# heathsc/bs_call

Hardware: AMD Instinct MI355X
Metric: genome positions called/sec (higher is better)
Workload: dtype f64

## Files before the change

### bs_call_amd/csrc/prepdev.hip

```cpp
#include <hip/hip_runtime.h>
#include <stdint.h>

#include "../../include/bscall_amd.h"

#define FLT_QUAL 63u

struct bsc_prep_plan {
  uint64_t src;
  uint64_t ms;
  uint32_t rl0;
  uint32_t w0, wl;
  uint32_t nm;
  uint32_t mark_l, mark_r;
  uint32_t out_len;
  uint32_t present;
  uint32_t trim_l, trim_r;
};

struct bsc_prep_desc {
  uint64_t srcw;
  uint32_t pk;
  int32_t pc;
};
#define PD_PRESENT 1u
#define PD_EDITED 2u
#define PD_SLOW 8u

#define PREP_CNT_WORDS 8u
#define PREP_CNT_SLOTS 64u
#define PE_ORI 1u
#define PE_READ 2u
#define PE_LIST 4u
#define PE_SOFT_POS 6u
#define PE_SOFT_ILL 7u
#define PE_INDEL 8u
#define PE_CAP 9u
#define PE_PROF_CAP 10u
#define PE_PROF_RANGE 11u

struct prep_rd {
  uint32_t w0, wl;
};
__device__ static __forceinline__ void d_left_trim(prep_rd &r, uint32_t l) {
  if (l > 0) {
    if (l >= r.wl) r.wl = 0;
    else {
      r.w0 += l;
      r.wl -= l;
    }
  }
}
__device__ static __forceinline__ void d_right_trim(prep_rd &r, uint32_t l) {
  if (l > 0) {
    if (l >= r.wl) r.wl = 0;
    else r.wl -= l;
  }
}

__device__ static __forceinline__ uint32_t d_qual(const uint8_t *sp, uint32_t i, uint32_t rl0, uint32_t mark_l, uint32_t mark_r) {
  return (i < mark_l || i >= rl0 - mark_r) ? FLT_QUAL : (uint32_t)sp[i] >> 2;
}

__device__ static __forceinline__ uint32_t d_ld32(const uint8_t *p);
__device__ static uint32_t d_mean_qual(const uint8_t *sp, const prep_rd &r, uint32_t rl0, uint32_t mark_l, uint32_t mark_r) {
  const uint32_t lo = r.w0 > mark_l ? r.w0 : mark_l;
  const uint32_t e0 = r.w0 + r.wl, e1 = rl0 - mark_r;
  const uint32_t hi = e0 < e1 ? e0 : e1;
  uint32_t tot = 0, n = 0, i = lo;
#define MQ_DWORD(w_)                                                                                                                   \
  {                                                                                                                                    \
    const uint32_t q = ((w_) >> 2) & 0x3f3f3f3fu;                                                                                      \
    const uint32_t nz = ((q ^ 0x3f3f3f3fu) + 0x7f7f7f7fu) & 0x80808080u;  \
    n += (uint32_t)__popc(nz);                                                                                                         \
    tot = __builtin_amdgcn_sad_u8(q & ((nz >> 7) * 0xffu), 0u, tot);                                       \
  }
  for (; i + 16u <= hi; i += 16u) {
    uint4 v;
    __builtin_memcpy(&v, sp + i, 16);
    MQ_DWORD(v.x) MQ_DWORD(v.y) MQ_DWORD(v.z) MQ_DWORD(v.w)
  }
  for (; i + 4u <= hi; i += 4u) MQ_DWORD(d_ld32(sp + i))
#undef MQ_DWORD
  for (; i < hi; i++) {
    const uint32_t q = (uint32_t)sp[i] >> 2;
// ... 291 lines not shown
    if (n_overlap) atomicAdd(&slot[1], n_overlap);
  }
}

__device__ static __forceinline__ uint32_t d_marked(const uint8_t *sp, uint32_t i, uint32_t rl0, uint32_t mark_l, uint32_t mark_r) {
  const bool in_r = i >= rl0 - mark_r;
  const uint32_t b = sp[(in_r && 2u * i > rl0 - 1u) ? rl0 - 1u - i : i];
  return (i < mark_l || in_r) ? (b & 3u) | (FLT_QUAL << 2) : (uint32_t)sp[i];
}

struct bsc_prep_prof {
  const uint8_t *ref;
  uint32_t x, n_ref, cap, used0;
  const uint32_t *used_scan;
  unsigned long long *table;
};
__device__ static const uint8_t PROF_REF[64] = {
    0, 0, 0, 0, 0, 0, 0, 0, 0, 0, 0, 8, 0, 0, 0, 0, 0, 4, 4, 0, 4, 0, 0, 0, 0, 0, 0, 8, 0, 0, 0, 0,
    0, 0, 0, 8, 0, 0, 0, 0, 0, 0, 0, 0, 0, 0, 0, 0, 0, 0, 0, 0, 0, 0, 0, 0, 0, 0, 0, 0, 0, 0, 0, 0};
__device__ static __forceinline__ uint32_t d_profile_base(uint32_t bs_strand, uint32_t c) {
  const uint32_t q = c >> 2;
  if (q < 20u  || q >= FLT_QUAL || bs_strand > 2u) return 0u;
  return ((bs_strand == 0 ? 0x7A6Bu : (bs_strand == 1 ? 0x5A4Bu : 0x7869u)) >> (4u * (c & 3u))) & 15u;
}

#define PREP_WAVES 4
#define PREP_BATCH 4u
#define PROF_LDS 512u

__device__ static __forceinline__ void d_prof_base(const bsc_prep_prof &F, uint32_t *s_prof, uint32_t strand, uint32_t used_t, int64_t v,
                                                   int32_t orig, uint32_t byte) {
  const uint32_t xx = d_profile_base(strand, byte);
  if (xx && v + 1 < (int64_t)F.n_ref) {
    const uint32_t ra = v >= 1 ? F.ref[v - 1] : 0u, rb = v >= 0 ? F.ref[v] : 0u, rc = F.ref[v + 1];
    const uint32_t m_before = PROF_REF[((ra << 3) | rb) & 63u], m_after = PROF_REF[((rb << 3) | rc) & 63u];
    if ((((xx & m_after) | ((xx & m_before) >> 1)) >> 2) & 1u) {
      const uint32_t ix = (uint32_t)(orig + 1);
      if (ix < used_t && ix < F.cap) {
        if (ix < PROF_LDS) atomicAdd(&s_prof[(xx & 3u) * PROF_LDS + ix], 1u);
        else atomicAdd(&F.table[(uint64_t)ix * 4u + (xx & 3u)], 1ull);
      }
    }
  }
}

__device__ static __forceinline__ uint32_t d_bcast(uint32_t v, uint32_t l) { return (uint32_t)__builtin_amdgcn_readlane((int)v, (int)l); }
__device__ static __forceinline__ unsigned long long d_bcast64(unsigned long long v, uint32_t l) {
  return (unsigned long long)d_bcast((uint32_t)v, l) | ((unsigned long long)d_bcast((uint32_t)(v >> 32), l) << 32);
}
__device__ static __forceinline__ uint32_t d_ld32(const uint8_t *p) {
  uint32_t v;
  __builtin_memcpy(&v, p, 4);
  return v;
}
__device__ static __forceinline__ void d_st32(uint8_t *p, uint32_t v) { __builtin_memcpy(p, &v, 4); }

struct prep_slow_ret {
  uint32_t c63, cge;
  uint32_t walked;
};

__device__ static __forceinline__ uint32_t prep_slow_src(const bsc_prep_plan &P, const bsc_misms *__restrict__ ms, bool edited, uint32_t j, bool &pad) {
  uint32_t s = j;
  pad = false;
  if (edited) {
    for (uint32_t z = P.nm; z-- > 0;) {
      const bsc_misms m = ms[z];
      if (m.type == BSC_MISMS_INS) {
        if (s >= m.position) {
          if (s - m.position < m.size) {
            pad = true;
            break;
          }
          s -= m.size;
        }
      } else if (m.type == BSC_MISMS_DEL) {
        if (s >= m.position) s += m.size;
      }
    }
  }
  return s;
}

__device__ __noinline__ static prep_slow_ret prep_slow_read(const bsc_prep_plan *__restrict__ plan_r, uint32_t flags, uint8_t *__restrict__ dp,
                                                            const uint8_t *__restrict__ seq, const bsc_misms *__restrict__ ms_work, uint32_t mq) {
  const unsigned lane = threadIdx.x & 63u;
  prep_slow_ret r = {0u, 0u, 0u};
  const bsc_prep_plan P = *plan_r;
  const uint8_t *const sp = seq + P.src;
  const bool edited = (flags & PD_EDITED) != 0;
  if (edited) {
    for (uint32_t s0 = 0; s0 < P.wl; s0 += 64u) {
      const uint32_t s = s0 + lane;
      if (s < P.wl) {
        const uint32_t q = d_marked(sp, P.w0 + s, P.rl0, P.mark_l, P.mark_r) >> 2;
        r.c63 += q == FLT_QUAL;
        r.cge += q >= mq;
      }
    }
  }
  const bsc_misms *const ms = ms_work + P.ms;
  bool walked = false;
  for (uint32_t j0 = 0; j0 < P.out_len; j0 += 64u) {
    const uint32_t j = j0 + lane;
    if (j < P.out_len) {
      bool pad;
      const uint32_t s = prep_slow_src(P, ms, edited, j, pad);
      const uint32_t byte = pad ? 0u : d_marked(sp, P.w0 + s, P.rl0, P.mark_l, P.mark_r);
      const uint32_t q = byte >> 2;
      if (!edited) {
        r.c63 += q == FLT_QUAL;
        r.cge += q >= mq;
      }
      walked |= q != 0 && q != FLT_QUAL;
      dp[j] = (uint8_t)byte;
    }
  }
  r.walked = __any(walked) ? 1u : 0u;
  return r;
}

__global__ __launch_bounds__(64 * PREP_WAVES) void bsc_prep_copy_kernel(const bsc_prep_plan *__restrict__ plan,
                                                                        const bsc_prep_desc *__restrict__ desc, uint32_t nr,
                                                                        const uint8_t *__restrict__ seq, const bsc_misms *__restrict__ ms_work,
                                                                        const unsigned long long *__restrict__ out_off, int32_t min_qual,
                                                                        bsc_template *__restrict__ tpl_out, uint8_t *__restrict__ seq_out,
                                                                        uint64_t seq_out_cap, unsigned long long *__restrict__ cnt) {
  const unsigned lane = threadIdx.x & 63u, lane4 = lane * 4u;
  const uint32_t wave = (uint32_t)__builtin_amdgcn_readfirstlane((int)(blockIdx.x * PREP_WAVES + (threadIdx.x >> 6)));
  const uint32_t n_waves = gridDim.x * PREP_WAVES;
  const uint32_t mq = min_qual < 0 ? 0u : (min_qual > 64 ? 64u : (uint32_t)min_qual), mq4 = mq * 0x01010101u;
  unsigned long long l_total = 0, l_bases = 0;
  uint32_t c63 = 0, cge = 0, l_reads = 0;
  const uint32_t n_reads2 = 2u * nr, n_groups = (n_reads2 + 63u) / 64u;
  for (uint32_t g = wave; g < n_groups; g += n_waves) {
    const uint32_t g0 = g * 64u, n = n_reads2 - g0 < 64u ? n_reads2 - g0 : 64u;
    const uint32_t ri = g0 + (lane < n ? lane : 0u), my_ti = ri >> 1, my_k = ri & 1u;
    bsc_prep_desc L = desc[ri];
    const unsigned long long l_off = out_off[ri];
    if (lane >= n) L.pk = 0;
    if (lane < n) {
      const uint32_t fl = L.pk >> 28;
      uint32_t ol = L.pk & 0xfffffu, wl = ol;
      if (fl & PD_SLOW) {
        ol = plan[ri].out_len;
        wl = plan[ri].wl;
      }
      tpl_out[my_ti].off[my_k] = l_off;
      if (l_off > seq_out_cap || seq_out_cap - l_off < ol) {
        atomicMin(&cnt[0], ((unsigned long long)my_ti << 8) | PE_CAP);
        L.pk &= 0xf0000000u;
      }
      l_total += (fl & PD_EDITED) ? wl : ol;
      if (fl & PD_PRESENT) {
        l_reads++;
        l_bases += wl;
      }
    }
    enum : uint32_t { KIND_LEAN = 1u, KIND_FAST = 2u, KIND_SLOW = 3u };
    const uint32_t my_len = L.pk & 0xfffffu, my_ml = (L.pk >> 20) & 0xffu;
    const uint32_t my_kind = my_len == 0 ? 0u : ((L.pk >> 28) & PD_SLOW ? KIND_SLOW : ((my_len <= 256u && my_ml == 0) ? KIND_LEAN : KIND_FAST));
    const uint32_t l_ctl = (L.pk & 0x0fffffffu) | (my_kind << 28) | (((L.pk >> 28) & PD_EDITED) ? 1u << 30 : 0u);
    const bool my_fetch = my_kind == KIND_LEAN || my_kind == KIND_FAST;
    const unsigned long long l_src = my_fetch ? (unsigned long long)(seq + L.srcw) - (unsigned long long)desc : 0ull;
    unsigned long long walked_mask = 0;
    const unsigned long long obase = d_bcast64(l_off, 0);
    const unsigned long long m_w0 = __ballot(my_kind == KIND_LEAN && my_len >= 16u && my_len <= 128u);
    const unsigned long long sbase = m_w0 ? d_bcast64(L.srcw, (uint32_t)__builtin_ctzll(m_w0)) : 0ull;
    const unsigned long long orel = l_off - obase, srel = L.srcw - sbase;
    const bool my_wide = my_kind == KIND_LEAN && my_len >= 16u && my_len <= 128u && orel < (1ull << 24) && srel < (1ull << 31);
    const uint32_t w_a = my_wide ? my_len | ((uint32_t)orel << 8) : 0u, w_s = my_wide ? (uint32_t)srel : 0u;
    const uint32_t l16 = (lane & 7u) * 16u, sub = lane & 56u;
    const uint8_t *const sp_w = seq + sbase;
    uint8_t *const dp_w = seq_out + obase;
    uint32_t walk_bits = 0;
    constexpr uint32_t RW = 2u;
    auto fetch8 = [&](uint32_t i0, uint4(&vv)[RW]) {
#pragma unroll
      for (uint32_t i = 0; i < RW; i++) {
        const int src = (int)(sub | ((i0 + i) & 7u));
        const uint32_t len = (uint32_t)__shfl((int)w_a, src) & 0xffu, so = (uint32_t)__shfl((int)w_s, src);
        const uint32_t last = len ? len - 16u : 0u;
        __builtin_memcpy(&vv[i], sp_w + (so + (l16 < last ? l16 : last)), 16);
      }
    };
    auto process8 = [&](const uint32_t i0, const uint4(&v)[RW]) {
#pragma unroll
      for (uint32_t i = 0; i < RW; i++) {
        const uint32_t l = i0 + i;
        const int src = (int)(sub | l);
        const uint32_t a_ = (uint32_t)__shfl((int)w_a, src), len = a_ & 0xffu;
        const bool act = l16 < len;
        const uint32_t o = l16 < len - 16u ? l16 : len - 16u, dup = act ? l16 - o : 16u;
        const uint32_t w4[4] = {v[i].x, v[i].y, v[i].z, v[i].w};
        uint32_t any = 0;
#pragma unroll
        for (uint32_t d = 0; d < 4u; d++) {
          const uint32_t ge = (((0x83828180u + 0x04040404u * d) - dup * 0x01010101u) >> 7) & 0x01010101u;
          const uint32_t wc = w4[d] & (ge * 0xffu);
          const uint32_t qh = ((wc >> 2) & 0x3f3f3f3fu) | 0x80808080u;
          const uint32_t q1 = qh + 0x01010101u;
          c63 += (uint32_t)__popc(q1 & 0x40404040u);
          cge += (uint32_t)__popc((qh - mq4) & 0x80808080u);
          any |= q1 & 0x3e3e3e3eu;
        }
        if (any) walk_bits |= 1u << l;
        if (act) __builtin_memcpy(dp_w + ((a_ >> 8) + o), &v[i], 16);
      }
    };
    auto one = [&](const uint32_t l) {
      const uint32_t k = l & 1u;
      const uint32_t ctl = d_bcast(l_ctl, l), kind = (ctl >> 28) & 3u, len = ctl & 0xfffffu;
      uint8_t *const dp = seq_out + d_bcast64(l_off, l);
      if (kind == KIND_SLOW) {
        const prep_slow_ret r = prep_slow_read(plan + g0 + l, (ctl >> 30) & 1u ? PD_EDITED : 0u, dp, seq, ms_work, mq);
        c63 += r.c63;
        cge += r.cge;
        if (k == 0 && r.walked) walked_mask |= 1ull << l;
        return;
      }
      const uint32_t ml = (ctl >> 20) & 0xffu;
      bool walked = false;
      for (uint32_t base = 0; base < len; base += 256u) {
        const uint32_t nominal = base + lane4;
        const bool act = nominal < len;
        const uint32_t o = nominal < len - 4u ? nominal : len - 4u;
        uint32_t w = act ? d_ld32((const uint8_t *)desc + d_bcast64(l_src, l) + o) : 0u;
        if (ml + 3u > base) {
          const uint32_t nmk = act && ml > o ? (ml - o < 4u ? ml - o : 4u) : 0u;
          const uint32_t mm = nmk >= 4u ? 0xffffffffu : (1u << (8u * nmk)) - 1u;
          w = (w & ~mm) | (((w & 0x03030303u) | 0xfcfcfcfcu) & mm);
        }
        const uint32_t wc = act ? w >> (8u * (nominal - o)) : 0u;
        const uint32_t qh = ((wc >> 2) & 0x3f3f3f3fu) | 0x80808080u;
        const uint32_t q1 = qh + 0x01010101u;
        c63 += (uint32_t)__popc(q1 & 0x40404040u);
        cge += (uint32_t)__popc((qh - mq4) & 0x80808080u);
        if (k == 0) walked |= __any((q1 & 0x3e3e3e3eu) != 0u) != 0;
        if (act) d_st32(dp + o, w);
      }
      if (k == 0 && walked) walked_mask |= 1ull << l;
    };
    if (__ballot(my_wide)) {
      uint4 va[RW], vb[RW];
      fetch8(0, va);
#pragma unroll
      for (uint32_t i0 = 0; i0 < 8u; i0 += 2u * RW) {
        fetch8(i0 + RW, vb);
        process8(i0, va);
        fetch8(i0 + 2u * RW, va);
        process8(i0 + RW, vb);
      }
      walk_bits |= (uint32_t)__shfl_xor((int)walk_bits, 1);
      walk_bits |= (uint32_t)__shfl_xor((int)walk_bits, 2);
      walk_bits |= (uint32_t)__shfl_xor((int)walk_bits, 4);
      walked_mask |= __ballot((walk_bits >> (lane & 7u)) & 1u);
    }
    for (unsigned long long rest = __ballot(my_kind != 0u && !my_wide); rest; rest &= rest - 1ull) one((uint32_t)__builtin_ctzll(rest));
    if (lane < n && my_k == 0) tpl_out[my_ti].flags = BSC_TPL_WALK_KNOWN | (((walked_mask >> lane) & 1ull) ? BSC_TPL_WALKED0 : 0u);
  }
  unsigned long long w[5] = {l_total, c63, cge, l_reads, l_bases};
  for (int i = 0; i < 5; i++)
    for (int o = 32; o > 0; o >>= 1) w[i] += __shfl_xor(w[i], o);
  if (mq == 0) w[2] = w[0];
  if (lane == 0) {
    const unsigned long long low = w[0] - w[2] - (mq > FLT_QUAL ? w[1] : 0ull), none = w[0] - w[1] - low;
    if (none) atomicAdd(&cnt[3], none);
    if (w[1]) atomicAdd(&cnt[4], w[1]);
    if (low) atomicAdd(&cnt[5], low);
    if (w[3]) atomicAdd(&cnt[6], w[3]);
    if (w[4]) atomicAdd(&cnt[7], w[4]);
  }
}

__global__ __launch_bounds__(256) void bsc_prep_refmask_kernel(const uint8_t *__restrict__ ref, uint32_t n_ref, uint8_t *__restrict__ mask) {
  const uint64_t i = ((uint64_t)blockIdx.x * 256u + threadIdx.x) * 4u;
  if (i >= (uint64_t)n_ref + 24u) return;
  uint32_t m = 0;
  if (i >= 12u && i - 8u + 7u <= n_ref) {
    const uint64_t v = i - 8u;
    const uint32_t lo = d_ld32(ref + v - 1u) & 0x07070707u, hi = d_ld32(ref + v + 3u) & 0x07070707u;
    const uint32_t r_at = __builtin_amdgcn_alignbyte(hi, lo, 1u), r_next = __builtin_amdgcn_alignbyte(hi, lo, 2u);
#define PROF_NE(x, c) ((((x) ^ ((c) * 0x01010101u)) + 0x7f7f7f7fu) & 0x80808080u)
    const uint32_t over_c = ~PROF_NE(r_at, 2u) & PROF_NE(r_next, 0u) & PROF_NE(r_next, 3u) & 0x80808080u;
    const uint32_t over_g = ~PROF_NE(r_at, 3u) & PROF_NE(lo, 0u) & PROF_NE(lo, 2u) & 0x80808080u;
#undef PROF_NE
    m = (over_c >> 5) | (over_g >> 4);
  } else {
    for (uint32_t t = 0; t < 4u; t++) {
      const uint64_t it = i + t;
      if (it >= 8u && it - 8u + 1u < n_ref) {
        const uint64_t v = it - 8u;
        const uint32_t ra = v >= 1 ? ref[v - 1] : 0u, rb = ref[v], rc = ref[v + 1];
        m |= ((PROF_REF[((rb << 3) | rc) & 63u] & 4u) | (PROF_REF[((ra << 3) | rb) & 63u] & 8u)) << (8u * t);
      }
    }
  }
  __builtin_memcpy(mask + i, &m, 4);
}

__global__ __launch_bounds__(64 * PREP_WAVES) void bsc_prep_profile_kernel(const bsc_prep_plan *__restrict__ plan, const bsc_prep_desc *__restrict__ desc,
                                                                           uint32_t nr, const bsc_misms *__restrict__ ms_work,
                                                                           const unsigned long long *__restrict__ out_off,
                                                                           const bsc_template *__restrict__ tpl_out, const uint8_t *__restrict__ seq_out,
                                                                           uint64_t seq_out_cap, unsigned long long *__restrict__ cnt,
                                                                           const uint8_t *__restrict__ mask, const bsc_prep_prof F) {
  __shared__ uint32_t s_prof[PROF_LDS * 4u];
  for (unsigned i = threadIdx.x; i < PROF_LDS * 4u; i += 64 * PREP_WAVES) s_prof[i] = 0;
  __syncthreads();
  const unsigned lane = threadIdx.x & 63u;
  const uint32_t wave = (uint32_t)__builtin_amdgcn_readfirstlane((int)(blockIdx.x * PREP_WAVES + (threadIdx.x >> 6)));
  const uint32_t n_waves = gridDim.x * PREP_WAVES;
  const uint32_t n_reads2 = 2u * nr, n_groups = (n_reads2 + 63u) / 64u;
  uint32_t acc[4][2] = {{0u, 0u}, {0u, 0u}, {0u, 0u}, {0u, 0u}};
  uint32_t acc_n = 0;
  bool acc_quarter = true;
  auto flush = [&]() {
    const uint32_t p0 = 8u * (acc_quarter ? (lane & 15u) : (lane & 31u));
#pragma unroll
    for (uint32_t b = 0; b < 4u; b++) {
      const uint32_t col = (0x63u >> (2u * b)) & 3u;
#pragma unroll
      for (uint32_t t = 0; t < 8u; t++) {
        const uint32_t c = (acc[b][t >> 2] >> (8u * (t & 3u))) & 0xffu;
        if (c) atomicAdd(&s_prof[col * PROF_LDS + p0 + t + 1u], c);
      }
      acc[b][0] = acc[b][1] = 0u;
    }
    acc_n = 0;
  };
  for (uint32_t g = wave; g < n_groups; g += n_waves) {
    const uint32_t g0 = g * 64u, n = n_reads2 - g0 < 64u ? n_reads2 - g0 : 64u;
    const uint32_t ri = g0 + (lane < n ? lane : 0u), my_ti = ri >> 1, my_k = ri & 1u;
    const bsc_prep_desc L = desc[ri];
    const unsigned long long l_off = out_off[ri];
    const uint32_t us_prev = my_ti ? F.used_scan[my_ti - 1u] : 0u, us_mine = F.used_scan[my_ti];
    const uint32_t t_strand = tpl_out[my_ti].bs_strand, t_pos = tpl_out[my_ti].pos[my_k];
    uint32_t c1 = 0, kind = 0, l_used = 0, l_strand = 0, l_ol = 0, top = 0;
    if (lane < n) {
      const uint32_t fl = L.pk >> 28;
      uint32_t ol = L.pk & 0xfffffu;
// ... 81 lines not shown
      };
      rnd ra[B], rb[B];
#pragma unroll
      for (uint32_t u = 0; u < B; u++) ask(u, ra[u]);
      for (uint32_t i0 = 0; i0 < rounds; i0 += 2u * B) {
        if (acc_n + 2u * B > 255u) flush();
#pragma unroll
        for (uint32_t u = 0; u < B; u++) ask(i0 + B + u, rb[u]);
#pragma unroll
        for (uint32_t u = 0; u < B; u++) count(u, ra[u]);
#pragma unroll
        for (uint32_t u = 0; u < B; u++) ask(i0 + 2u * B + u, ra[u]);
#pragma unroll
        for (uint32_t u = 0; u < B; u++) count(B + u, rb[u]);
        acc_n += 2u * B;
      }
    }
    unsigned long long m_long = __ballot(kind == 2u);
    while (m_long) {
      const uint32_t l = (uint32_t)__builtin_ctzll(m_long);
      m_long &= m_long - 1ull;
      const uint32_t ol = d_bcast(l_ol, l), k = l & 1u, strand = d_bcast(l_strand, l), used_t = d_bcast(l_used, l);
      const int32_t pc = (int32_t)d_bcast((uint32_t)L.pc, l);
      const int64_t v0 = (int64_t)d_bcast(c1, l) - 1;
      const uint8_t *const dp = seq_out + d_bcast64(l_off, l);
      const bool slow = (d_bcast(L.pk, l) >> 28) & PD_SLOW;
      bsc_prep_plan P;
      bool edited = false;
      if (slow) {
        P = plan[g0 + l];
        edited = (d_bcast(L.pk, l) >> 28) & PD_EDITED;
      }
      for (uint32_t jb = 0; jb < ol; jb += 64u) {
        const uint32_t j = jb + lane;
        if (j < ol) {
          bool pad = false;
          const uint32_t s = slow ? prep_slow_src(P, ms_work + P.ms, edited, j, pad) : j;
          if (!pad) d_prof_base(F, s_prof, strand, used_t, v0 + j, k ? pc - (int32_t)s : pc + (int32_t)s, dp[j]);
        }
      }
    }
  }
  flush();
  __syncthreads();
  for (unsigned i = threadIdx.x; i < PROF_LDS * 4u; i += 64 * PREP_WAVES)
    if (s_prof[i] && i % PROF_LDS < F.cap) atomicAdd(&F.table[(uint64_t)(i % PROF_LDS) * 4u + i / PROF_LDS], (unsigned long long)s_prof[i]);
}

extern "C" int bsc_dev_scan_u64(const void *in, void *out, uint32_t n, void *tmp, size_t tmp_bytes, void *stream);

extern "C" size_t bsc_dev_prep_plan_bytes(void) { return sizeof(bsc_prep_plan) + sizeof(bsc_prep_desc); }

extern "C" int bsc_dev_scan_max_u32(const void *in, void *out, uint32_t n, void *tmp, size_t tmp_bytes, void *stream);

extern "C" int bsc_dev_launch_prep(const void *raw, uint32_t nr, const void *seq, uint64_t seq_bytes, const void *misms, uint64_t n_misms,
                                   const bsc_prep_params *par, void *ms_work, void *plan, void *out_len, void *out_off, void *scan_tmp,
                                   size_t scan_tmp_bytes, void *tpl_out, void *seq_out, uint64_t seq_out_cap, void *cnt, int num_cus,
                                   void *stream, const void *prof_ref, uint32_t prof_x, uint32_t prof_n_ref, uint32_t prof_cap,
                                   uint32_t prof_used0, void *prof_table, void *max_pos1, void *used_scan, void *prof_mask) {
  hipStream_t s = (hipStream_t)stream;
  bsc_prep_desc *const desc = (bsc_prep_desc *)((bsc_prep_plan *)plan + 2ull * nr);
  if (!nr) return (int)hipMemsetAsync(out_off, 0, sizeof(unsigned long long), s);
  hipError_t e = hipMemsetAsync((unsigned long long *)out_len + 2ull * nr, 0, sizeof(unsigned long long), s);
  if (e != hipSuccess) return (int)e;
  hipLaunchKernelGGL(bsc_prep_plan_kernel, dim3((nr + 255u) / 256u), dim3(256), 0, s, (const bsc_raw_template *)raw, nr, (const uint8_t *)seq,
                     seq_bytes, (const bsc_misms *)misms, n_misms, *par, (bsc_misms *)ms_work, (bsc_prep_plan *)plan, desc,
                     (unsigned long long *)out_len, (bsc_template *)tpl_out, (unsigned long long *)cnt, prof_ref ? (uint32_t *)max_pos1 : nullptr);
  if ((e = hipGetLastError()) != hipSuccess) return (int)e;
  int rc = bsc_dev_scan_u64(out_len, out_off, 2u * nr + 1u, scan_tmp, scan_tmp_bytes, stream);
  if (rc) return rc;
  bsc_prep_prof F = {nullptr, 0u, 0u, 0u, 0u, nullptr, nullptr};
  if (prof_ref) {
    if ((rc = bsc_dev_scan_max_u32(max_pos1, used_scan, nr, scan_tmp, scan_tmp_bytes, stream))) return rc;
    F.ref = (const uint8_t *)prof_ref;
    F.x = prof_x;
    F.n_ref = prof_n_ref;
    F.cap = prof_cap;
    F.used0 = prof_used0;
    F.used_scan = (const uint32_t *)used_scan;
    F.table = (unsigned long long *)prof_table;
  }
  unsigned g = ((nr + 31u) / 32u + PREP_WAVES - 1u) / PREP_WAVES;
  static int per_cu[2] = {0, 0};
  for (int pv = 0; pv < (prof_ref ? 2 : 1); pv++)
    if (!per_cu[pv]) {
      int nb = 0;
      const hipError_t eo = pv ? hipOccupancyMaxActiveBlocksPerMultiprocessor(&nb, bsc_prep_profile_kernel, 64 * PREP_WAVES, 0)
                               : hipOccupancyMaxActiveBlocksPerMultiprocessor(&nb, bsc_prep_copy_kernel, 64 * PREP_WAVES, 0);
      per_cu[pv] = (eo == hipSuccess && nb > 0) ? nb : 4;
      (void)hipGetLastError();
    }
  unsigned gc = g, gp = g;
  if (gc > (unsigned)num_cus * (unsigned)per_cu[0]) gc = (unsigned)num_cus * (unsigned)per_cu[0];
  hipLaunchKernelGGL(bsc_prep_copy_kernel, dim3(gc), dim3(64 * PREP_WAVES), 0, s, (const bsc_prep_plan *)plan, (const bsc_prep_desc *)desc, nr,
                     (const uint8_t *)seq, (const bsc_misms *)ms_work, (const unsigned long long *)out_off, par->min_qual, (bsc_template *)tpl_out,
                     (uint8_t *)seq_out, seq_out_cap, (unsigned long long *)cnt);
  if ((e = hipGetLastError()) != hipSuccess) return (int)e;
  if (prof_ref) {
    hipLaunchKernelGGL(bsc_prep_refmask_kernel, dim3((unsigned)(((uint64_t)prof_n_ref + 24u + 1023u) / 1024u)), dim3(256), 0, s, (const uint8_t *)prof_ref,
                       prof_n_ref, (uint8_t *)prof_mask);
    if ((e = hipGetLastError()) != hipSuccess) return (int)e;
    if (gp > (unsigned)num_cus * (unsigned)per_cu[1]) gp = (unsigned)num_cus * (unsigned)per_cu[1];
    hipLaunchKernelGGL(bsc_prep_profile_kernel, dim3(gp), dim3(64 * PREP_WAVES), 0, s, (const bsc_prep_plan *)plan, (const bsc_prep_desc *)desc, nr,
                       (const bsc_misms *)ms_work, (const unsigned long long *)out_off, (const bsc_template *)tpl_out, (const uint8_t *)seq_out,
                       seq_out_cap, (unsigned long long *)cnt, (const uint8_t *)prof_mask, F);
  }
  return (int)hipGetLastError();
}
```

### bs_call_amd/csrc/kernels.hip

```cpp
#include <hip/hip_runtime.h>
#include <stdint.h>

#include "bsmath.h"
#include "callmath.h"
#include "devtables.h"
#include "synth.h"

#ifndef TILE
#define TILE 256
#endif
#ifndef BSC_TILES_PER_WAVE
#define BSC_TILES_PER_WAVE 16
#endif
#ifndef BSC_WAVES_PER_SIMD
#define BSC_WAVES_PER_SIMD 4
#endif

template <bool FULL>
__global__ __launch_bounds__(TILE, BSC_WAVES_PER_SIMD) void bsc_call_kernel_t(const uint32_t *__restrict__ cts,
                                                                      const uint8_t *__restrict__ ref,
                                                                      uint64_t n_sites, uint64_t wt_begin,
                                                                      uint64_t wt_end, uint32_t *__restrict__ out,
                                                                      uint32_t out_dw, uint8_t *__restrict__ skip,
                                                                      const bsc_dev_tables *__restrict__ tb,
                                                                      uint32_t *__restrict__ het_list,
                                                                      unsigned long long *__restrict__ counters) {
  __shared__ __attribute__((aligned(16))) uint32_t lds_slot[TILE / 64][SLOT_DW];
  __shared__ double s_k[44], s_lnk[44], s_half[44], s_one[44];
#ifdef BSC_TABLES_GLOBAL
  const double *const s_logtab = tb->log_tab;
  const unsigned long long *const s_exptab = tb->exp_tab;
#else
  __shared__ double s_logtab[256];
  __shared__ unsigned long long s_exptab[256];
#endif
  __shared__ unsigned int s_cnt[12];
  __shared__ double s_ptab[PT_WORDS];
  __shared__ uint8_t s_pairs[TILE / 64][256];

  const unsigned tid = threadIdx.x;
  const unsigned lane = tid & 63u;
  const unsigned wid = __builtin_amdgcn_readfirstlane(tid >> 6);
  if (tid < 44) {
    s_k[tid] = tb->k[tid];
    s_lnk[tid] = tb->ln_k[tid];
    s_half[tid] = tb->ln_k_half[tid];
    s_one[tid] = tb->ln_k_one[tid];
  }
#ifndef BSC_TABLES_GLOBAL
  for (unsigned i = tid; i < 256; i += TILE) {
    s_logtab[i] = tb->log_tab[i];
    s_exptab[i] = tb->exp_tab[i];
  }
#endif
  if (tid < 12) s_cnt[tid] = 0;
  const double l = 1.0 - tb->under_conv;
  const double t = tb->over_conv;
  const double lrb = tb->lrb, lrb1 = tb->lrb1;
  __syncthreads();
  for (unsigned i = tid; i < PT_WORDS; i += TILE) s_ptab[i] = pure_log_entry(i, l, t, s_k, s_logtab);
  __syncthreads();

  uint32_t *slot = lds_slot[wid];
  const uint32_t wave_stride = gridDim.x * (TILE / 64);
  const uint32_t wt_last = (uint32_t)wt_end;
  for (uint32_t wt = (uint32_t)wt_begin + blockIdx.x * (TILE / 64) + wid; wt < wt_last; wt += wave_stride) {
    const uint64_t site0 = (uint64_t)wt * 64;
    const unsigned nvalid = FULL ? 64u : (unsigned)((n_sites - site0) < 64 ? (n_sites - site0) : 64);
    const bool full = FULL;
    const uint64_t site = site0 + lane;
    const bool valid = FULL || lane < nvalid;
    const unsigned rf = valid ? ref[site] : 0u;

    uint32_t w[IN_DW];
    if (full) {
      const char *src = reinterpret_cast<const char *>(cts + site0 * IN_DW) + lane * 16;
#pragma unroll
      for (int j = 0; j < 6; j++) dma16(src + j * 1024, slot + j * 256);
      if (lane < 32) dma16(src + 6 * 1024, slot + 6 * 256);
      asm volatile("s_waitcnt vmcnt(0)" ::: "memory");
      const uint2 *rec = reinterpret_cast<const uint2 *>(slot + lane * IN_DW);
#pragma unroll
      for (int i = 0; i < IN_DW / 2; i++) {
        const uint2 v = rec[i];
        w[2 * i] = v.x;
        w[2 * i + 1] = v.y;
      }
    } else {
#pragma unroll
      for (int i = 0; i < IN_DW; i++) w[i] = valid ? cts[site * IN_DW + i] : 0u;
    }
#include "call_body.inc"
    const bool het = covered && ((0x16Eu >> mxi) & 1u);
    if (covered) {
      atomicAdd(&s_cnt[0], 1u);
      atomicAdd(&s_cnt[1 + mxi], 1u);
    }
    {
      const unsigned long long m = __ballot(het);
      if (lane == 0) {
        reinterpret_cast<unsigned long long *>(het_list)[wt] = m;
        if (m) atomicAdd(&s_cnt[11], (unsigned)__popcll(m));
      }
    }
    if (valid) skip[site] = covered ? 0 : 1;

#pragma unroll 1
    for (unsigned half = 0; half < 2; half++) {
      __builtin_amdgcn_wave_barrier();
      const bool mine = valid && (lane >> 5) == half;
      auto write_record = [&](auto *rec) {
        if (covered) {
#pragma unroll
          for (int j = 0; j < 8; j++) rec[j] = make_uint2(cnt[j], 0u);
          rec[8] = make_uint2(qpack0 & 0xffu, (qpack0 >> 8) & 0xffu);
          rec[9] = make_uint2((qpack0 >> 16) & 0xffu, qpack0 >> 24);
          rec[10] = make_uint2(qpack1 & 0xffu, (qpack1 >> 8) & 0xffu);
          rec[11] = make_uint2((qpack1 >> 16) & 0xffu, qpack1 >> 24);
#pragma unroll
          for (int g = 0; g < 10; g++) {
            const uint64_t b = bsm_bits(gp[g]);
            rec[12 + g] = make_uint2((uint32_t)b, (uint32_t)(b >> 32));
          }
          rec[22] = make_uint2(0u, 0u);
          rec[23] = make_uint2((uint32_t)mq, (uint32_t)aq);
          rec[24] = make_uint2((uint32_t)mxi, 0u);
        } else {
#pragma unroll
          for (int j = 0; j < 25; j++) rec[j] = make_uint2(0u, 0u);
        }
        if (out_dw > OUT_DW) rec[25] = make_uint2(covered ? 0u : 0x100u, 0u);
      };
      if (mine) {
        if (full) write_record(reinterpret_cast<uint2 *>(slot + (lane & 31u) * out_dw));
        else write_record(reinterpret_cast<uint2 *>(out + site * out_dw));
      }
      if (full) {
        __builtin_amdgcn_wave_barrier();
        const unsigned nvec = 32u * out_dw / 4u;
        uint4 *dst = reinterpret_cast<uint4 *>(out + (site0 + half * 32u) * out_dw);
        const uint4 *srcv = reinterpret_cast<const uint4 *>(slot);
#pragma unroll
        for (unsigned v = 0; v < 7; v++) {
          const unsigned idx = v * 64u + lane;
          if (idx < nvec) {
            typedef unsigned int u32x4 __attribute__((ext_vector_type(4)));
            __builtin_nontemporal_store(reinterpret_cast<const u32x4 *>(srcv)[idx], reinterpret_cast<u32x4 *>(dst) + idx);
          }
        }
      }
    }
  }

  __syncthreads();
  if (tid < 12 && s_cnt[tid]) atomicAdd(&counters[BSC_CNT_COVERED + tid], (unsigned long long)s_cnt[tid]);
}

#define FI_THREADS 256
#define FI_LIST 2048
extern "C" __global__ __launch_bounds__(FI_THREADS) void bsc_fisher_kernel(const uint32_t *__restrict__ cts,
                                                                           uint32_t *__restrict__ out, uint32_t out_dw,
                                                                           const bsc_dev_tables *__restrict__ tb,
                                                                           const unsigned long long *__restrict__ masks,
                                                                           uint32_t n_tiles, uint32_t chunk_tiles) {
  __shared__ double s_lf[256];
  __shared__ double s_logtab[256];
  __shared__ unsigned long long s_exptab[256];
  __shared__ uint32_t s_scan[FI_THREADS + 1];
  __shared__ uint32_t s_list[FI_LIST];
  const unsigned tid = threadIdx.x;
  s_lf[tid] = tb->lfact[tid];
  s_logtab[tid] = tb->log_tab[tid];
  s_exptab[tid] = tb->exp_tab[tid];
  const uint32_t per = (chunk_tiles + FI_THREADS - 1) / FI_THREADS;
  for (uint32_t c0 = blockIdx.x * chunk_tiles; c0 < n_tiles; c0 += gridDim.x * chunk_tiles) {
    const uint32_t c1 = min(c0 + chunk_tiles, n_tiles);
    const uint32_t t0 = min(c0 + tid * per, c1), t1 = min(t0 + per, c1);
    uint32_t mine = 0;
    for (uint32_t t = t0; t < t1; t++) mine += (uint32_t)__popcll(masks[t]);
    __syncthreads();
    s_scan[tid + 1] = mine;
    if (tid == 0) s_scan[0] = 0;
    __syncthreads();
    if (tid < 64) {
      uint32_t a = s_scan[4 * tid + 1], b = a + s_scan[4 * tid + 2], c = b + s_scan[4 * tid + 3], d = c + s_scan[4 * tid + 4];
      uint32_t run = d;
#pragma unroll
      for (int off = 1; off < 64; off <<= 1) {
        const uint32_t v = __shfl_up(run, off);
        if ((int)tid >= off) run += v;
      }
      const uint32_t base = run - d;
      s_scan[4 * tid + 1] = base + a;
      s_scan[4 * tid + 2] = base + b;
      s_scan[4 * tid + 3] = base + c;
      s_scan[4 * tid + 4] = base + d;
    }
    __syncthreads();
    const uint32_t total = s_scan[FI_THREADS], first = s_scan[tid];
    for (uint32_t w0 = 0; w0 < total; w0 += FI_LIST) {
      if (w0) __syncthreads();
      if (first < w0 + FI_LIST && first + mine > w0) {
        uint32_t k = first;
        for (uint32_t t = t0; t < t1; t++) {
          unsigned long long m = masks[t];
          while (m) {
            const unsigned bit = (unsigned)__builtin_ctzll(m);
            m &= m - 1ull;
            if (k >= w0 && k < w0 + FI_LIST) s_list[k - w0] = t * 64u + bit;
            k++;
          }
        }
      }
      __syncthreads();
      const uint32_t cnt = min((uint32_t)FI_LIST, total - w0);
      for (uint32_t i = tid; i < cnt; i += FI_THREADS) {
        const uint64_t site = s_list[i];
        const uint32_t *p = cts + site * IN_DW;
        uint32_t f[8], r[8];
#pragma unroll
        for (int j = 0; j < 8; j++) {
          f[j] = p[j];
          r[j] = p[8 + j];
        }
        uint32_t *rec = out + site * out_dw;
        const unsigned mxi = rec[48] & 0xffu;
        int t0_, t1_, t2_, t3_;
        strand_table(mxi, f, r, t0_, t1_, t2_, t3_);
        double z = fisher_dev(t0_, t1_, t2_, t3_, s_lf, s_logtab, (const uint64_t *)s_exptab);
        if (z < 1.0e-20) z = 1.0e-20;
        const double fs = bsm_log_t(z, s_logtab) / BSM_LN10;
        const uint64_t b = bsm_bits(fs);
        reinterpret_cast<uint2 *>(rec)[22] = make_uint2((uint32_t)b, (uint32_t)(b >> 32));
      }
    }
  }
}

extern "C" __global__ __launch_bounds__(256) void bsc_synth_kernel(uint64_t seed, uint64_t first_site, uint64_t n,
                                                                   uint32_t coverage, uint32_t flags,
                                                                   uint32_t *__restrict__ cts,
                                                                   uint8_t *__restrict__ ref) {
  for (uint64_t i = (uint64_t)blockIdx.x * blockDim.x + threadIdx.x; i < n; i += (uint64_t)gridDim.x * blockDim.x) {
    uint32_t counts[16], nr, rf;
    float q[8], m2;
    syn_site(seed, first_site + i, coverage, flags, counts, &nr, q, &m2, &rf);
    uint32_t *p = cts + i * IN_DW;
#pragma unroll
    for (int j = 0; j < 16; j++) p[j] = counts[j];
    p[16] = nr;
#pragma unroll
    for (int j = 0; j < 8; j++) p[17 + j] = __float_as_uint(q[j]);
    p[25] = __float_as_uint(m2);
    ref[i] = (uint8_t)rf;
  }
}


extern "C" int bsc_dev_launch_call(const void *cts, const void *ref, uint64_t n, void *out, uint32_t out_dw, void *skip,
                                   const void *tb, void *het_list, void *counters, int num_cus, void *stream,
                                   void *ev_start, void *ev_mid, void *ev_stop) {
  if (n == 0) return 0;
  hipStream_t s = (hipStream_t)stream;
  if (ev_start) (void)hipEventRecord((hipEvent_t)ev_start, s);
  uint64_t resident = (uint64_t)num_cus * (BSC_WAVES_PER_SIMD * 4) / (TILE / 64);
  if (resident < 1) resident = 1;
  const uint64_t n_full = n / 64;
  hipError_t e = hipSuccess;
  if (n_full) {
    const uint64_t n_tiles = (n_full + (TILE / 64) - 1) / (TILE / 64);
    uint64_t rounds = n_full / (resident * (TILE / 64) * BSC_TILES_PER_WAVE);
    rounds = rounds < 1 ? 1 : (rounds > 16 ? 16 : rounds);
    uint64_t grid = resident * rounds;
    if (grid > n_tiles) grid = n_tiles;
    hipLaunchKernelGGL(bsc_call_kernel_t<true>, dim3((unsigned)grid), dim3(TILE), 0, s, (const uint32_t *)cts,
                       (const uint8_t *)ref, n, (uint64_t)0, n_full, (uint32_t *)out, out_dw, (uint8_t *)skip,
                       (const bsc_dev_tables *)tb, (uint32_t *)het_list, (unsigned long long *)counters);
    e = hipGetLastError();
    if (e != hipSuccess) return (int)e;
  }
  if (n & 63u) {
    hipLaunchKernelGGL(bsc_call_kernel_t<false>, dim3(1), dim3(TILE), 0, s, (const uint32_t *)cts, (const uint8_t *)ref, n,
                       n_full, n_full + 1, (uint32_t *)out, out_dw, (uint8_t *)skip, (const bsc_dev_tables *)tb,
                       (uint32_t *)het_list, (unsigned long long *)counters);
    e = hipGetLastError();
    if (e != hipSuccess) return (int)e;
  }
  if (ev_mid) (void)hipEventRecord((hipEvent_t)ev_mid, s);
  {
    const uint32_t n_tiles = (uint32_t)((n + 63) / 64);
    const uint32_t grid = (uint32_t)num_cus * 2u;
    uint32_t chunk = (n_tiles + grid - 1) / grid;
    chunk = chunk < 64u ? 64u : (chunk > 4096u ? 4096u : chunk);
    const uint32_t n_chunks = (n_tiles + chunk - 1) / chunk;
    hipLaunchKernelGGL(bsc_fisher_kernel, dim3(n_chunks < grid ? n_chunks : grid), dim3(FI_THREADS), 0, s, (const uint32_t *)cts,
                       (uint32_t *)out, out_dw, (const bsc_dev_tables *)tb, (const unsigned long long *)het_list, n_tiles, chunk);
  }
  e = hipGetLastError();
  if (ev_stop) (void)hipEventRecord((hipEvent_t)ev_stop, s);
  return (int)e;
}

extern "C" int bsc_dev_launch_synth(uint64_t seed, uint64_t first_site, uint64_t n, uint32_t coverage, uint32_t flags,
                                    void *cts, void *ref, int num_cus, void *stream) {
  if (n == 0) return 0;
  uint64_t grid = (n + 255) / 256;
  const uint64_t cap = (uint64_t)num_cus * 32u;
  if (grid > cap) grid = cap;
  hipLaunchKernelGGL(bsc_synth_kernel, dim3((unsigned)grid), dim3(256), 0, (hipStream_t)stream, seed, first_site, n,
                     coverage, flags, (uint32_t *)cts, (uint8_t *)ref);
  return (int)hipGetLastError();
}
```

Baseline: 16.75 billion.

## Stage per-wave output bytes in LDS and flush with aligned nontemporal stores

Each wave now assembles its group's output sequence bytes in a per-wave LDS image instead of scattering unaligned 4- and 16-byte global stores. After the group is built, the image is written to global memory in aligned 16-byte nontemporal chunks, with byte-wise handling at the edges. The host sizes the stage buffer from the mean read length and available LDS, and recomputes occupancy for the grid. The kernel also gains a waves-per-EU attribute and sched barriers. This costs LDS, may reduce occupancy, and adds a wave-level flush pass.

```diff
diff --git a/bs_call_amd/csrc/prepdev.hip b/bs_call_amd/csrc/prepdev.hip
--- a/bs_call_amd/csrc/prepdev.hip
+++ b/bs_call_amd/csrc/prepdev.hip
@@ -1,5 +1,7 @@
 #include <hip/hip_runtime.h>
 #include <stdint.h>
+
+#include <type_traits>
 
 #include "../../include/bscall_amd.h"
 
@@ -457,7 +459,15 @@
   return s;
 }
 
-__device__ __noinline__ static prep_slow_ret prep_slow_read(const bsc_prep_plan *__restrict__ plan_r, uint32_t flags, uint8_t *__restrict__ dp,
+extern __shared__ uint4 s_prep_stage[];
+#define PREP_NO_IMG 0xffffffffu
+#define PREP_LDS __attribute__((address_space(3)))
+typedef PREP_LDS uint8_t prep_lds_u8;
+typedef uint32_t __attribute__((aligned(1))) prep_u32_any;
+typedef unsigned int prep_u32x4 __attribute__((ext_vector_type(4)));
+typedef prep_u32x4 __attribute__((aligned(1))) prep_u32x4_any;
+
+__device__ __noinline__ static prep_slow_ret prep_slow_read(const bsc_prep_plan *__restrict__ plan_r, uint32_t flags, uint8_t *__restrict__ dp, uint32_t img,
                                                             const uint8_t *__restrict__ seq, const bsc_misms *__restrict__ ms_work, uint32_t mq) {
   const unsigned lane = threadIdx.x & 63u;
   prep_slow_ret r = {0u, 0u, 0u};
@@ -488,20 +498,24 @@
         r.cge += q >= mq;
       }
       walked |= q != 0 && q != FLT_QUAL;
-      dp[j] = (uint8_t)byte;
+      if (img != PREP_NO_IMG) ((prep_lds_u8 *)s_prep_stage)[img + j] = (uint8_t)byte;
+      else dp[j] = (uint8_t)byte;
     }
   }
   r.walked = __any(walked) ? 1u : 0u;
   return r;
 }
 
-__global__ __launch_bounds__(64 * PREP_WAVES) void bsc_prep_copy_kernel(const bsc_prep_plan *__restrict__ plan,
+__global__ __launch_bounds__(64 * PREP_WAVES) __attribute__((amdgpu_waves_per_eu(6))) void bsc_prep_copy_kernel(const bsc_prep_plan *__restrict__ plan,
                                                                         const bsc_prep_desc *__restrict__ desc, uint32_t nr,
                                                                         const uint8_t *__restrict__ seq, const bsc_misms *__restrict__ ms_work,
                                                                         const unsigned long long *__restrict__ out_off, int32_t min_qual,
                                                                         bsc_template *__restrict__ tpl_out, uint8_t *__restrict__ seq_out,
-                                                                        uint64_t seq_out_cap, unsigned long long *__restrict__ cnt) {
+                                                                        uint64_t seq_out_cap, unsigned long long *__restrict__ cnt,
+                                                                        uint32_t stage_bytes) {
   const unsigned lane = threadIdx.x & 63u, lane4 = lane * 4u;
+  const uint32_t img0 = (threadIdx.x >> 6) * stage_bytes;
+  prep_lds_u8 *const img = (prep_lds_u8 *)s_prep_stage + img0;
   const uint32_t wave = (uint32_t)__builtin_amdgcn_readfirstlane((int)(blockIdx.x * PREP_WAVES + (threadIdx.x >> 6)));
   const uint32_t n_waves = gridDim.x * PREP_WAVES;
   const uint32_t mq = min_qual < 0 ? 0u : (min_qual > 64 ? 64u : (uint32_t)min_qual), mq4 = mq * 0x01010101u;
@@ -540,6 +554,10 @@
     const unsigned long long l_src = my_fetch ? (unsigned long long)(seq + L.srcw) - (unsigned long long)desc : 0ull;
     unsigned long long walked_mask = 0;
     const unsigned long long obase = d_bcast64(l_off, 0);
+    const unsigned long long gend = out_off[g0 + n];
+    const uint32_t ia = (uint32_t)((unsigned long long)(seq_out + obase) & 15ull);
+    const bool staged = __builtin_amdgcn_readfirstlane((int)(gend <= seq_out_cap && gend >= obase && gend - obase + ia <= stage_bytes)) != 0;
+    const uint32_t span = staged ? (uint32_t)(gend - obase) : 0u;
     const unsigned long long m_w0 = __ballot(my_kind == KIND_LEAN && my_len >= 16u && my_len <= 128u);
     const unsigned long long sbase = m_w0 ? d_bcast64(L.srcw, (uint32_t)__builtin_ctzll(m_w0)) : 0ull;
     const unsigned long long orel = l_off - obase, srel = L.srcw - sbase;
@@ -559,7 +577,8 @@
         __builtin_memcpy(&vv[i], sp_w + (so + (l16 < last ? l16 : last)), 16);
       }
     };
-    auto process8 = [&](const uint32_t i0, const uint4(&v)[RW]) {
+    auto process8 = [&](auto st, const uint32_t i0, const uint4(&v)[RW]) {
+      constexpr bool ST = decltype(st)::value;
 #pragma unroll
       for (uint32_t i = 0; i < RW; i++) {
         const uint32_t l = i0 + i;
@@ -580,15 +599,21 @@
           any |= q1 & 0x3e3e3e3eu;
         }
         if (any) walk_bits |= 1u << l;
-        if (act) __builtin_memcpy(dp_w + ((a_ >> 8) + o), &v[i], 16);
+        if (act) {
+          if (ST) *(PREP_LDS prep_u32x4_any *)(img + (ia + (a_ >> 8) + o)) = prep_u32x4{v[i].x, v[i].y, v[i].z, v[i].w};
+          else __builtin_memcpy(dp_w + ((a_ >> 8) + o), &v[i], 16);
+        }
       }
     };
     auto one = [&](const uint32_t l) {
       const uint32_t k = l & 1u;
       const uint32_t ctl = d_bcast(l_ctl, l), kind = (ctl >> 28) & 3u, len = ctl & 0xfffffu;
-      uint8_t *const dp = seq_out + d_bcast64(l_off, l);
+      const unsigned long long off_l = d_bcast64(l_off, l);
+      uint8_t *const dp = seq_out + off_l;
+      prep_lds_u8 *const ip = img + (ia + (uint32_t)(off_l - obase));
       if (kind == KIND_SLOW) {
-        const prep_slow_ret r = prep_slow_read(plan + g0 + l, (ctl >> 30) & 1u ? PD_EDITED : 0u, dp, seq, ms_work, mq);
+        const prep_slow_ret r = prep_slow_read(plan + g0 + l, (ctl >> 30) & 1u ? PD_EDITED : 0u, dp,
+                                               staged ? img0 + ia + (uint32_t)(off_l - obase) : PREP_NO_IMG, seq, ms_work, mq);
         c63 += r.c63;
         cge += r.cge;
         if (k == 0 && r.walked) walked_mask |= 1ull << l;
@@ -612,26 +637,47 @@
         c63 += (uint32_t)__popc(q1 & 0x40404040u);
         cge += (uint32_t)__popc((qh - mq4) & 0x80808080u);
         if (k == 0) walked |= __any((q1 & 0x3e3e3e3eu) != 0u) != 0;
-        if (act) d_st32(dp + o, w);
+        if (act) {
+          if (staged) *(PREP_LDS prep_u32_any *)(ip + o) = w;
+          else d_st32(dp + o, w);
+        }
       }
       if (k == 0 && walked) walked_mask |= 1ull << l;
     };
-    if (__ballot(my_wide)) {
+    auto wide = [&](auto st) {
       uint4 va[RW], vb[RW];
       fetch8(0, va);
 #pragma unroll
       for (uint32_t i0 = 0; i0 < 8u; i0 += 2u * RW) {
         fetch8(i0 + RW, vb);
-        process8(i0, va);
+        process8(st, i0, va);
+        __builtin_amdgcn_sched_barrier(0);
         fetch8(i0 + 2u * RW, va);
-        process8(i0 + RW, vb);
-      }
+        process8(st, i0 + RW, vb);
+        __builtin_amdgcn_sched_barrier(0);
+      }
+    };
+    __builtin_amdgcn_wave_barrier();
+    if (__ballot(my_wide)) {
+      if (staged) wide(std::true_type{});
+      else wide(std::false_type{});
       walk_bits |= (uint32_t)__shfl_xor((int)walk_bits, 1);
       walk_bits |= (uint32_t)__shfl_xor((int)walk_bits, 2);
       walk_bits |= (uint32_t)__shfl_xor((int)walk_bits, 4);
       walked_mask |= __ballot((walk_bits >> (lane & 7u)) & 1u);
     }
     for (unsigned long long rest = __ballot(my_kind != 0u && !my_wide); rest; rest &= rest - 1ull) one((uint32_t)__builtin_ctzll(rest));
+    if (staged) {
+      __builtin_amdgcn_wave_barrier();
+      const uint32_t iend = ia + span;
+      uint8_t *const gp = seq_out + obase - ia;
+#pragma unroll 1
+      for (uint32_t p = lane * 16u; p < iend; p += 1024u) {
+        if (p >= ia && p + 16u <= iend) __builtin_nontemporal_store(*(const PREP_LDS prep_u32x4 *)(img + p), reinterpret_cast<prep_u32x4 *>(gp + p));
+        else
+          for (uint32_t q = p > ia ? p : ia; q < p + 16u && q < iend; q++) gp[q] = img[q];
+      }
+    }
     if (lane < n && my_k == 0) tpl_out[my_ti].flags = BSC_TPL_WALK_KNOWN | (((walked_mask >> lane) & 1ull) ? BSC_TPL_WALKED0 : 0u);
   }
   unsigned long long w[5] = {l_total, c63, cge, l_reads, l_bases};
@@ -879,6 +925,7 @@
   }
   unsigned g = ((nr + 31u) / 32u + PREP_WAVES - 1u) / PREP_WAVES;
   static int per_cu[2] = {0, 0};
+  static int lds_cu = 0;
   for (int pv = 0; pv < (prof_ref ? 2 : 1); pv++)
     if (!per_cu[pv]) {
       int nb = 0;
@@ -887,11 +934,37 @@
       per_cu[pv] = (eo == hipSuccess && nb > 0) ? nb : 4;
       (void)hipGetLastError();
     }
+  if (!lds_cu) {
+    int dv = 0, v = 0;
+    if (hipGetDevice(&dv) != hipSuccess || hipDeviceGetAttribute(&v, hipDeviceAttributeMaxSharedMemoryPerMultiprocessor, dv) != hipSuccess || v < 65536) v = 65536;
+    lds_cu = v;
+    (void)hipGetLastError();
+  }
+  const uint64_t mean_len = (seq_bytes + 2ull * nr - 1ull) / (2ull * nr);
+  const uint64_t need = 64ull * mean_len + 2ull * mean_len + 32ull;
+  uint32_t stage = 16u;
+  for (int w = per_cu[0]; w >= 1; w--) {
+    uint32_t sw = ((uint32_t)lds_cu / (uint32_t)w / PREP_WAVES) & ~511u;
+    if (sw > 65536u / PREP_WAVES) sw = 65536u / PREP_WAVES;
+    if (sw >= need) {
+      stage = sw;
+      break;
+    }
+  }
+  static uint32_t occ_stage = 0;
+  static int occ_blocks = 0;
+  if (occ_stage != stage) {
+    int nb = 0;
+    const hipError_t eo = hipOccupancyMaxActiveBlocksPerMultiprocessor(&nb, bsc_prep_copy_kernel, 64 * PREP_WAVES, (size_t)stage * PREP_WAVES);
+    occ_blocks = (eo == hipSuccess && nb > 0) ? nb : 4;
+    occ_stage = stage;
+    (void)hipGetLastError();
+  }
   unsigned gc = g, gp = g;
-  if (gc > (unsigned)num_cus * (unsigned)per_cu[0]) gc = (unsigned)num_cus * (unsigned)per_cu[0];
-  hipLaunchKernelGGL(bsc_prep_copy_kernel, dim3(gc), dim3(64 * PREP_WAVES), 0, s, (const bsc_prep_plan *)plan, (const bsc_prep_desc *)desc, nr,
-                     (const uint8_t *)seq, (const bsc_misms *)ms_work, (const unsigned long long *)out_off, par->min_qual, (bsc_template *)tpl_out,
-                     (uint8_t *)seq_out, seq_out_cap, (unsigned long long *)cnt);
+  if (gc > (unsigned)num_cus * (unsigned)occ_blocks) gc = (unsigned)num_cus * (unsigned)occ_blocks;
+  hipLaunchKernelGGL(bsc_prep_copy_kernel, dim3(gc), dim3(64 * PREP_WAVES), (size_t)stage * PREP_WAVES, s, (const bsc_prep_plan *)plan,
+                     (const bsc_prep_desc *)desc, nr, (const uint8_t *)seq, (const bsc_misms *)ms_work, (const unsigned long long *)out_off, par->min_qual,
+                     (bsc_template *)tpl_out, (uint8_t *)seq_out, seq_out_cap, (unsigned long long *)cnt, stage);
   if ((e = hipGetLastError()) != hipSuccess) return (int)e;
   if (prof_ref) {
     hipLaunchKernelGGL(bsc_prep_refmask_kernel, dim3((unsigned)(((uint64_t)prof_n_ref + 24u + 1023u) / 1024u)), dim3(256), 0, s, (const uint8_t *)prof_ref,
```

Result: no change. 16.75 billion, median of 2 (+0.0%).

## Software-prefetch next tile into registers and run one persistent grid round

Applied to the files above, without the earlier changes.

Replaces the synchronous global-to-LDS copy plus vmcnt(0) wait with a register prefetch of the next tile's pile-up data and reference base. The prefetch is issued right after the current tile is read from LDS and deposited into LDS once the outputs are written, so load latency overlaps the call math. To make room for the extra prefetch registers, waves per SIMD drops to 3, the grid is capped at a single persistent round, and the half loop is unrolled. The cost is register pressure and lower occupancy, with fewer waves left to hide latency.

```diff
diff --git a/bs_call_amd/csrc/kernels.hip b/bs_call_amd/csrc/kernels.hip
--- a/bs_call_amd/csrc/kernels.hip
+++ b/bs_call_amd/csrc/kernels.hip
@@ -12,8 +12,11 @@
 #ifndef BSC_TILES_PER_WAVE
 #define BSC_TILES_PER_WAVE 16
 #endif
+#ifndef BSC_MAX_ROUNDS
+#define BSC_MAX_ROUNDS 1
+#endif
 #ifndef BSC_WAVES_PER_SIMD
-#define BSC_WAVES_PER_SIMD 4
+#define BSC_WAVES_PER_SIMD 3
 #endif
 
 template <bool FULL>
@@ -61,24 +64,42 @@
   for (unsigned i = tid; i < PT_WORDS; i += TILE) s_ptab[i] = pure_log_entry(i, l, t, s_k, s_logtab);
   __syncthreads();
 
-  uint32_t *slot = lds_slot[wid];
+  typedef unsigned int u32x4 __attribute__((ext_vector_type(4)));
   const uint32_t wave_stride = gridDim.x * (TILE / 64);
   const uint32_t wt_last = (uint32_t)wt_end;
-  for (uint32_t wt = (uint32_t)wt_begin + blockIdx.x * (TILE / 64) + wid; wt < wt_last; wt += wave_stride) {
+  uint32_t wt = (uint32_t)wt_begin + blockIdx.x * (TILE / 64) + wid;
+  uint32_t *slot = lds_slot[wid];
+  u32x4 pf[7];
+  unsigned rf_next = 0;
+  auto fetch_tile = [&](uint32_t tile) {
+    const uint64_t nsite0 = (uint64_t)tile * 64;
+    const u32x4 *nsrc = reinterpret_cast<const u32x4 *>(cts + nsite0 * IN_DW) + lane;
+    rf_next = ref[nsite0 + lane];
+#pragma unroll
+    for (int j = 0; j < 6; j++) pf[j] = __builtin_nontemporal_load(nsrc + j * 64);
+    if (lane < 32) pf[6] = __builtin_nontemporal_load(nsrc + 6 * 64);
+  };
+  auto deposit_tile = [&]() {
+    u32x4 *dstv = reinterpret_cast<u32x4 *>(slot) + lane;
+#pragma unroll
+    for (int j = 0; j < 6; j++) dstv[j * 64] = pf[j];
+    if (lane < 32) dstv[6 * 64] = pf[6];
+  };
+  if (FULL && wt < wt_last) {
+    fetch_tile(wt);
+    deposit_tile();
+  }
+  for (; wt < wt_last; wt += wave_stride) {
     const uint64_t site0 = (uint64_t)wt * 64;
     const unsigned nvalid = FULL ? 64u : (unsigned)((n_sites - site0) < 64 ? (n_sites - site0) : 64);
     const bool full = FULL;
     const uint64_t site = site0 + lane;
     const bool valid = FULL || lane < nvalid;
-    const unsigned rf = valid ? ref[site] : 0u;
+    const unsigned rf = FULL ? rf_next : (valid ? ref[site] : 0u);
+    const bool have_next = FULL && wt + wave_stride < wt_last;
 
     uint32_t w[IN_DW];
     if (full) {
-      const char *src = reinterpret_cast<const char *>(cts + site0 * IN_DW) + lane * 16;
-#pragma unroll
-      for (int j = 0; j < 6; j++) dma16(src + j * 1024, slot + j * 256);
-      if (lane < 32) dma16(src + 6 * 1024, slot + 6 * 256);
-      asm volatile("s_waitcnt vmcnt(0)" ::: "memory");
       const uint2 *rec = reinterpret_cast<const uint2 *>(slot + lane * IN_DW);
 #pragma unroll
       for (int i = 0; i < IN_DW / 2; i++) {
@@ -86,6 +107,7 @@
         w[2 * i] = v.x;
         w[2 * i + 1] = v.y;
       }
+      if (have_next) fetch_tile(wt + wave_stride);
     } else {
 #pragma unroll
       for (int i = 0; i < IN_DW; i++) w[i] = valid ? cts[site * IN_DW + i] : 0u;
@@ -105,7 +127,7 @@
     }
     if (valid) skip[site] = covered ? 0 : 1;
 
-#pragma unroll 1
+#pragma unroll
     for (unsigned half = 0; half < 2; half++) {
       __builtin_amdgcn_wave_barrier();
       const bool mine = valid && (lane >> 5) == half;
@@ -143,12 +165,15 @@
 #pragma unroll
         for (unsigned v = 0; v < 7; v++) {
           const unsigned idx = v * 64u + lane;
-          if (idx < nvec) {
-            typedef unsigned int u32x4 __attribute__((ext_vector_type(4)));
+          if (v < 6 || idx < nvec) {
             __builtin_nontemporal_store(reinterpret_cast<const u32x4 *>(srcv)[idx], reinterpret_cast<u32x4 *>(dst) + idx);
           }
         }
       }
+    }
+    if (FULL) {
+      if (!have_next) break;
+      deposit_tile();
     }
   }
 
@@ -270,7 +295,7 @@
   if (n_full) {
     const uint64_t n_tiles = (n_full + (TILE / 64) - 1) / (TILE / 64);
     uint64_t rounds = n_full / (resident * (TILE / 64) * BSC_TILES_PER_WAVE);
-    rounds = rounds < 1 ? 1 : (rounds > 16 ? 16 : rounds);
+    rounds = rounds < 1 ? 1 : (rounds > BSC_MAX_ROUNDS ? BSC_MAX_ROUNDS : rounds);
     uint64_t grid = resident * rounds;
     if (grid > n_tiles) grid = n_tiles;
     hipLaunchKernelGGL(bsc_call_kernel_t<true>, dim3((unsigned)grid), dim3(TILE), 0, s, (const uint32_t *)cts,
```

Measured after the change: 16.68 billion positions/s before, 15.58 billion positions/s after. 6.5% lower.
